# TencentYoutuResearch/ImageMatching-OETR

Hardware: AMD Instinct MI355X
Metric: image-pairs/sec @640x640 (OETR hot path: feature correlation + overlap regression, features resident in HBM) (higher is better)
Workload: dtype f32 (3xf16-split operands, fp32 accumulate); 1 GPU; BASELINE configs[1]: batch=8 pairs/GPU, 640x640 -> 20x20 tokens/image, C=256, 8 enc + 2 dec layers, f32_split_f16; pairs_per_gpu=8, global_pairs=8, streams=3, world_size=1, gpu_max_hw_queues=4, encoder_tile_rows=64, tail_mode=direct form (throughput setting for overlapped streams), parallelism=pairs sharded over 1 rank(s); all-gather of boxes only

## Files before the change

imagematching_oetr_amd/csrc/api.hip:

```cpp
#include <math.h>
#include <stdlib.h>
#include <string.h>

#include <string>
#include <vector>

#include "../../include/oetr_hip.h"
#include "common.h"

using namespace oetr;

constexpr int OETR_PREREDUCE_MIN_TOKENS = 768;
constexpr int OETR_DIRECT_TAIL_MIN_ROWS = 16000;

namespace {

thread_local std::string g_err;

oetr_status fail(oetr_status st, const std::string& msg) {
  g_err = msg;
  return st;
}
oetr_status hip_fail(hipError_t e, const char* what) {
  return fail(OETR_ERR_HIP, std::string(what) + ": " + hipGetErrorString(e));
// ... 97 lines not shown
    "k_decoder", "k_heat_conv", "k_heat_final", "k_size_reg", "k_boxes", "k_decoder_convp",
    "k_heat_combine", "k_neck_proj", "k_neck_conv", "k_neck_out", "k_kv_reduce"};

struct oetr_trace {
  std::vector<hipEvent_t> ev;
  std::vector<int> kid;
  int used = 0;
  int dropped = 0;
};

struct oetr_ctx {
  oetr_trace* trace = nullptr;
  int device = 0;
  int mode = GM_SPLIT;
  int kv_prereduce = -1;
  mutable int dec_fault = 0;
  int dec_split = 0;
  int tail_mode = 0;
  int policy = 0;
  int enc_tile = 0;
  int attn_full = 0;
  int num_cus = 256;
  float* dev = nullptr;
  size_t dev_floats = 0;
  EncLayerDev enc[OETR_N_ENC];
  DecKVDev dkv;
  DecLayerDev dec[OETR_N_DEC];
  const float* qe[2];
  const float *dec_tgt1, *dec_q0, *dec_qkv1;
  HeadsDev heads;
// ... 194 lines not shown

oetr_status run_correlation(oetr_ctx* h, const Geom& g, const Workspace& w, const float* feat1,
                            const float* feat2, const float* pos1, const float* pos2,
                            int enc_layers, hipStream_t s, bool with_decoder = true,
                            bool resident = false, const float* mask1 = nullptr,
                            const float* mask2 = nullptr) {
  EncLaunch p;
  memset(&p, 0, sizeof(p));
  if (!resident) {
    p.feat_nchw[0] = feat1; p.feat_nchw[1] = feat2;
    p.pos_nchw[0] = pos1; p.pos_nchw[1] = pos2;
    p.pos_out = w.pos;
  }
  p.tile_rows = encoder_tile_rows(h, g);
  p.g = encoder_geom(g, p.tile_rows);
#ifdef OETR_ABLATE
  { const char* e = getenv("OETR_ABLATE"); p.dbg = e ? atoi(e) : 0; }
#endif
#ifdef OETR_PHASE_TIMING
  {
    static long long* tb = nullptr;
    if (!tb) (void)hipMalloc(&tb, sizeof(long long) * 16 * 65536);
    p.tbuf = tb;
    g_tbuf = tb;
  }
#endif
  p.x = w.x; p.qp = w.qp; p.pos = w.pos;
  p.mask[0] = mask1; p.mask[1] = mask2;
  p.flags = w.flags;
  p.attn_full = h->attn_full;
  p.policy = h->policy;
  for (int i = 0; i < 2; ++i) p.lpad[i] = g.nt[i] * TM;
  p.vt_off[0] = 0; p.vt_off[1] = (size_t)g.N * C * p.lpad[0];
  p.kbuf_out = w.kbuf[0]; p.vt_out = w.vt[0];
  p.a = h->enc[0];
  p.kv_out = w.kvp[0]; p.ks_out = w.ksp[0];
  int prereduce = h->attn_full ? 0 : h->kv_prereduce;
  if (prereduce < 0) prereduce = (g.L[0] >= OETR_PREREDUCE_MIN_TOKENS || g.L[1] >= OETR_PREREDUCE_MIN_TOKENS) ? 1 : 0;
  TRACED(h, s, K_ENC_A, launch_encoder(p, false, 0, h->mode, s));
  p.feat_nchw[0] = p.feat_nchw[1] = p.pos_nchw[0] = p.pos_nchw[1] = nullptr;
  for (int l = 0; l < enc_layers; ++l) {
    p.b = h->enc[l];
    p.b_cross = l & 1;
    p.kv_in = w.kvp[l & 1]; p.ks_in = w.ksp[l & 1];
    p.kv_reduced = 0;
// ... 992 lines not shown
  (void)hipGetDevice(&prev);
  hipError_t e = hipSetDevice(device);
  if (e == hipSuccess) e = measure_mfma_rate(prop.multiProcessorCount, seconds, tflops, static_cast<hipStream_t>(stream));
  (void)hipSetDevice(prev);
  if (e != hipSuccess) return hip_fail(e, "oetr_debug_mfma_rate");
  return OETR_OK;
}

oetr_status oetr_set_state_prereduce(oetr_handle h, int on) {
  if (!h) return fail(OETR_ERR_BAD_ARG, "oetr_set_state_prereduce: NULL handle");
  if (on < -1 || on > 1) return fail(OETR_ERR_BAD_ARG, "oetr_set_state_prereduce: -1 (auto), 0 (off) or 1 (a reduction launch between the encoder launches)");
  h->kv_prereduce = on;
  return OETR_OK;
}

oetr_status oetr_set_attention(oetr_handle h, oetr_attention mode) {
  if (!h) return fail(OETR_ERR_BAD_ARG, "oetr_set_attention: NULL handle");
  if (mode != OETR_ATTENTION_LINEAR && mode != OETR_ATTENTION_FULL)
    return fail(OETR_ERR_BAD_ARG, "oetr_set_attention: unknown mode");
  if (mode == OETR_ATTENTION_FULL && h->policy != 0)
    return fail(OETR_ERR_UNSUPPORTED, "attention 'full' is not built for OETR_DTYPE_F32_SPLIT_QK16");
  if (mode == OETR_ATTENTION_FULL && !gm_f16_range(h->mode) && h->mode != GM_F32)
    return fail(OETR_ERR_UNSUPPORTED, "attention 'full' is built for OETR_DTYPE_F32_SPLIT_F16, OETR_DTYPE_F16 and OETR_DTYPE_F32");
  h->attn_full = mode == OETR_ATTENTION_FULL;
  return OETR_OK;
}

oetr_status oetr_set_trace(oetr_handle h, oetr_trace_handle t) {
  if (!h) return fail(OETR_ERR_BAD_ARG, "oetr_set_trace: NULL handle");
  h->trace = t;
// ... 39 lines not shown
```

imagematching_oetr_amd/csrc/common.h:

```cpp
#pragma once
#include <hip/hip_runtime.h>
#include <stdint.h>

#include <string>
#include <type_traits>

#include "../../include/oetr_hip.h"

namespace oetr {

constexpr int C = 256;
constexpr int NH = 8;
constexpr int HD = 32;
constexpr int FF = 512;
constexpr int TM = 32;
constexpr int LDA = C + 4;
constexpr int LDH = FF + 4;
constexpr int NTHREADS = 256;
constexpr int KV_FLOATS = NH * HD * HD;
constexpr float LN_EPS = 1e-5f;
constexpr float ATTN_EPS = 1e-6f;
constexpr int MAX_TOKENS = 10000;


// ... 818 lines not shown
  float* z0_out;
  float* dkv1_out;
  float* dks1_out;
  const float* dec_q0;
  EncLayerDev b;
  EncLayerDev a;
  DecKVDev d;
  int attn_full;
  const float* kbuf_in;
  const float* vt_in;
  float* kbuf_out;
  float* vt_out;
  int lpad[2];
  size_t vt_off[2];
  int tile_rows;
  int b_cross;
  int kv_reduced;
  int policy;
  int dbg;
  long long* tbuf;
  uint32_t* flags;
  const float* feat_nchw[2];
  const float* pos_nchw[2];
  float* pos_out;
  const float* mask[2];
};

hipError_t launch_encoder(const EncLaunch& p, bool has_b, int tail, int mode, hipStream_t s);
hipError_t launch_kv_reduce(const Geom& g, const float* kvp, const float* ksp, float* kvr, float* ksr,
                            hipStream_t s);

struct MhaDev {
  const float *wq_t, *wk_t, *wv_t, *wm_t;
  const float *bq, *bk, *bv;
};
struct DecLayerDev {
  MhaDev self_attn, cross;
  const float *w1_t, *w2_t;
  const float *n1w, *n1b, *n2w, *n2b, *n3w, *n3b;
};
struct DecLaunch {
  Geom g;
  DecLayerDev layer[2];
// ... 124 lines not shown
```

imagematching_oetr_amd/csrc/encoder.hip:

```cpp
#include <type_traits>

#include "common.h"


#ifndef OETR_SOAK_AMP
#define OETR_SOAK_AMP 0
#endif
#ifndef OETR_SPLIT_STATE
#define OETR_SPLIT_STATE 1
#endif

namespace oetr {

constexpr int S0_OFF = 0;
constexpr int S1_OFF = S0_OFF + TM * LDA;
constexpr int H_OFF = S1_OFF + TILE_FLOATS;
constexpr int KSUM_OFF = H_OFF + HID_FLOATS;
constexpr int Z_OFF = KSUM_OFF + C;
constexpr int LNP_OFF = Z_OFF + TM * NH;
constexpr int SMEM_FLOATS = LNP_OFF + 6 * C;

template <int NW>
struct EncCfg {
  static constexpr int NT = 8 / NW;
// ... 58 lines not shown
}

template <int THREADS>
__device__ __forceinline__ void load_tile(float* S, const float* __restrict__ src, int nvalid,
                                          int tid) {
#pragma unroll
  for (int i = 0; i < (TM * C / 4) / THREADS; ++i) {
    const int idx = tid + THREADS * i;
    const int r = idx >> 6, c4 = idx & 63;
    *reinterpret_cast<f32x4*>(S + r * LDA + 4 * c4) =
        reinterpret_cast<const f32x4*>(src + (size_t)min(r, nvalid - 1) * C)[c4];
  }
}

template <int THREADS, int ROWS>
__device__ __forceinline__ void load_tile_nchw(float* S, const float* __restrict__ src, int L,
                                               int nvalid, int tid) {
  constexpr int CG = THREADS / ROWS;
  const int r = tid % ROWS, cg = tid / ROWS;
  const float* s = src + min(r, nvalid - 1);
#pragma unroll
  for (int i = 0; i < C / CG; ++i) {
    const int c = cg + CG * i;
    S[r * LDA + c] = s[(size_t)c * L];
  }
}
template <int THREADS, int ROWS>
__device__ __forceinline__ void store_tile_tokens(float* __restrict__ dst, const float* S, int nvalid,
                                                  int tid) {
#pragma unroll
  for (int i = 0; i < (ROWS * C / 4) / THREADS; ++i) {
    const int idx = tid + THREADS * i;
    const int r = idx >> 6, c4 = idx & 63;
    if (r < nvalid)
      reinterpret_cast<f32x4*>(dst + (size_t)r * C)[c4] = *reinterpret_cast<const f32x4*>(S + r * LDA + 4 * c4);
  }
}

template <int MODE>
__device__ __forceinline__ void full_attention_tile(const EncLaunch& p, int n, int ss, size_t row_base,
// ... 594 lines not shown
    dec_layer(std::integral_constant<int, 1>{});
  }
  range_report<MODE>(rg, p.flags);
}

constexpr int LNX_LD = 36;
template <int RTW>
struct E2 {
  static constexpr int RFL = (2 * RTW * LDAH * 2 + 3) / 4;
  static_assert(RFL >= RTW * LDA, "region holds the f32 tile too");
  static constexpr int R1 = 0, R2 = RFL, KSUM = 2 * RFL, LNP = KSUM + C;
  static constexpr int LNX = LNP + 6 * C;
  static constexpr int SMEM = LNX + RTW * LNX_LD;
};

template <int MODE, int NMT = 2, bool MASKED = false>
__device__ __forceinline__ void kv_state_64(const f32x16 (&accK)[NMT], const f32x16 (&accV)[NMT],
                                            int S_len, int nvalid, int half, bool two, f32x16& kv,
                                            float& ksum, Range& rg, const float* msk_s = nullptr) {
  const float inv_len = 1.0f / (float)S_len;
  kv = f32x16{0};
  ksum = 0.f;
  int nv2 = nvalid - 4 * half;
  asm volatile("" : "+v"(nv2));
  if constexpr (MODE == GM_SPLIT && OETR_SPLIT_STATE) {
    f32x16 c1 = {0};
#if OETR_SOAK_AMP & 2
    __builtin_amdgcn_s_setprio(3);
#endif
    auto row_tile = [&](auto MT_) {
      constexpr int mt = decltype(MT_)::value;
#pragma unroll
      for (int st = 0; st < 2; ++st) {
        f32x4 k0, k1, v0, v1;
#pragma unroll
        for (int i = 0; i < 8; ++i) {
          const int r = 8 * st + i;
          float m;
          if constexpr (MASKED) m = msk_s[32 * mt + crow(r, half)];
          else m = 32 * mt + crow(r, 0) < nv2 ? 1.0f : 0.0f;
          const float kk = elu1(accK[mt][r]) * m;
          const float vv = accV[mt][r] * (inv_len * m);
          ksum += kk;
          if (i < 4) { k0[i] = kk; v0[i] = vv; } else { k1[i - 4] = kk; v1[i - 4] = vv; }
        }
        f32x4 ah, al, bh, bl;
        split8(k0, k1, ah, al, rg);
        split8(v0, v1, bh, bl, rg);
        mma16_split3(ah, al, bh, bl, kv, c1);
        __builtin_amdgcn_sched_barrier(0);
      }
    };
    row_tile(std::integral_constant<int, 0>{});
    if constexpr (NMT == 2) {
      if (two) row_tile(std::integral_constant<int, 1>{});
    }
#if OETR_SOAK_AMP & 2
    __builtin_amdgcn_s_setprio(0);
#endif
#pragma unroll
    for (int r = 0; r < 16; ++r) kv[r] = fmaf(c1[r], SPLIT_INV, kv[r]);
  } else {
    auto row_tile = [&](auto MT_) {
      constexpr int mt = decltype(MT_)::value;
      auto operands = [&](int r, float& k, float& v) {
        float m;
        if constexpr (MASKED) m = msk_s[32 * mt + crow(r, half)];
        else m = 32 * mt + crow(r, 0) < nv2 ? 1.0f : 0.0f;
        const float x = accK[mt][r];
        k = (elu1(x)) * m;
        ksum += k;
        v = accV[mt][r] * (inv_len * m);
      };
      float kc, vc;
      operands(0, kc, vc);
#pragma unroll
      for (int r = 0; r < 16; ++r) {
        float kn = 0.f, vn = 0.f;
        if (r + 1 < 16) operands(r + 1, kn, vn);
        kv = __builtin_amdgcn_mfma_f32_32x32x2f32(kc, vc, kv, 0, 0, 0);
        __builtin_amdgcn_sched_barrier(0);
        kc = kn; vc = vn;
// ... 4 lines not shown
      if (two) row_tile(std::integral_constant<int, 1>{});
    }
  }
  ksum += __shfl_xor(ksum, 32, 64);
}
__device__ __forceinline__ void kv_state_write(const f32x16& kv, float ksum, int lane, int wave,
                                               float* __restrict__ kv_out,
                                               float* __restrict__ ks_out, int slot) {
  f32x4* dst = reinterpret_cast<f32x4*>(kv_out) + ((size_t)slot * NH + wave) * 4 * 64;
#pragma unroll
  for (int q = 0; q < 4; ++q) {
    f32x4 o = {kv[4 * q], kv[4 * q + 1], kv[4 * q + 2], kv[4 * q + 3]};
    store16(reinterpret_cast<float*>(dst), (q * 64 + (unsigned)lane) * 16u, o);
  }
  if (lane < 32) (ks_out + (size_t)slot * C + wave * HD)[(unsigned)lane] = ksum;
}

template <bool HAS_B, int TAIL, int MODE, int POL, int ROWS, int RTW = RT, bool MASKED = false>
__device__ __forceinline__ void encoder64_body(const EncLaunch& p, float* smem) {
  constexpr int NMT = RTW / 32, THREADS = 512, TPR = THREADS / RTW, F4 = 64 / TPR;
  using L2 = E2<RTW>;
  using SP = SitePolicy<POL>;
  float* R1f = smem + L2::R1;
  float* R2f = smem + L2::R2;
  Range rg;
  const PlanesT<MODE, RTW> P1(R1f, &rg), P2(R2f, &rg);
  float* Xf = HAS_B ? R2f : R1f;
  float* ksum_s = smem + L2::KSUM;
  float* lnp_s = smem + L2::LNP;
  float* lnx_s = smem + L2::LNX;
  using WS = WStream2T<MODE, ROWS, NMT>;
  WS ws;
  constexpr int P_MERGE = 0;
  constexpr int P_1A = WS::adv(P_MERGE), P_1B = WS::adv(P_1A), P_2A = WS::adv(P_1B), P_2B = WS::adv(P_2A);
  constexpr int P_T0 = HAS_B ? WS::adv(P_2B) : 0;
  constexpr int P_T1 = WS::adv(P_T0), P_T2 = WS::adv(P_T1), P_T3 = WS::adv(P_T2);

  const Geom& g = p.g;
  const int tid = threadIdx.x, lane = tid & 63, wave = __builtin_amdgcn_readfirstlane(tid >> 6);
  const int half = lane >> 5, col = lane & 31;
  const int wcol = 32 * wave;
  const int lrow = tid / TPR, lpart = tid % TPR;

  const int logical = xcd_remap(blockIdx.x, g.ntiles);
  const int per = g.nt[0] + g.nt[1];
  const int n = logical / per;
  const int rem = logical - n * per;
  const int side = rem >= g.nt[0];
  const int t_idx = side ? rem - g.nt[0] : rem;
  const int L = g.L[side];
  const int l0 = t_idx * RTW;
  const int nvalid = min(RTW, L - l0);
  const size_t row_base = (size_t)g.row0[side] + (size_t)n * L + l0;
  const int slot = g.tile0[side] + n * g.nt[side] + t_idx;
  const size_t qrow_base = (size_t)slot * RTW;
  const bool nchw = !HAS_B && p.feat_nchw[0] != nullptr;
  ws.set_rows(nvalid);
  ws.set_lane(lane);

  stage_ln_params<THREADS, HAS_B, TAIL>(lnp_s, p, tid);
  const f32x4* pos = reinterpret_cast<const f32x4*>(
                         p.pos + (size_t)(g.prow0[side] + l0 + min(lrow, nvalid - 1)) * C) + lpart;

  f32x16 xacc[NMT];
  PHASE_STAMP(p, 0);
  if (!HAS_B) PHASE_STAMP(p, 13);

  if (HAS_B) {
    const int ss = p.b_cross ? 1 - side : side;
    const int S_len = g.L[ss];
    const int nts = p.kv_reduced ? 1 : g.nt[ss];
    const int src_slot0 = p.kv_reduced ? ss * g.N + n : g.tile0[ss] + n * g.nt[ss];

    f32x4 kvB[4];
#pragma unroll
    for (int q = 0; q < 4; ++q) kvB[q] = f32x4{0.f, 0.f, 0.f, 0.f};
    {
      constexpr int KVR = 7;
      const unsigned ln = lane, kl = tid & (C - 1);
      const f32x4* kvp = reinterpret_cast<const f32x4*>(p.kv_in) + ((size_t)src_slot0 * NH + wave) * 256;
      const float* ksp = p.ks_in + (size_t)src_slot0 * C;
      float ks = 0.f;
      if (nts == 1) {
#pragma unroll
        for (int e = 0; e < 4; ++e) kvB[e] = kvp[e * 64 + ln];
        ks = ksp[kl];
      } else
      for (int ti0 = 0; ti0 < nts; ti0 += KVR) {
        f32x4 tmp[KVR][4];
// ... 3 lines not shown
          const int ti = min(ti0 + u, nts - 1);
#pragma unroll
          for (int e = 0; e < 4; ++e) tmp[u][e] = kvp[(size_t)ti * (NH * 256) + e * 64 + ln];
          kt[u] = ksp[(size_t)ti * C + kl];
        }
#pragma unroll
        for (int u = 0; u < KVR; ++u)
          if (ti0 + u < nts) {
#pragma unroll
            for (int e = 0; e < 4; ++e) kvB[e] += tmp[u][e];
            ks += kt[u];
          }
      }
      if (tid < C) ksum_s[tid] = ks;
    }
    ws.template prime<C, P_MERGE, SP::MERGE>(p.b.wmerge, p.b.wmerge_l, wave, 0, lane);
    f32x4 qfrag[NMT][4];
    {
      const f32x4* qf = reinterpret_cast<const f32x4*>(p.qp + qrow_base * C) + (size_t)wave * NMT * 4 * 64;
#pragma unroll
      for (int mt = 0; mt < NMT; ++mt)
#pragma unroll
        for (int u = 0; u < 4; ++u) qfrag[mt][u] = qf[(mt * 4 + u) * 64 + (unsigned)lane];
    }
#pragma unroll
    for (int mt = 0; mt < NMT; ++mt) {
      const float* xr = p.x + (row_base + min(32 * mt + col, nvalid - 1)) * C + wcol + 4 * half;
#pragma unroll
      for (int g4 = 0; g4 < 4; ++g4) {
        const f32x4 v = *reinterpret_cast<const f32x4*>(xr + 8 * g4);
#pragma unroll
        for (int i = 0; i < 4; ++i) xacc[mt][4 * g4 + i] = v[i];
      }
    }
    __syncthreads();
    PHASE_STAMP(p, 1);

    {
      f32x4 kvh[2], kvl[2], ksh[2], ksl[2];
      const float inv_S = 1.0f / (float)S_len;
      (void)inv_S;
      if constexpr (gm_f16_range(MODE)) {
#pragma unroll
        for (int s2 = 0; s2 < 2; ++s2) {
          split8(kvB[2 * s2], kvB[2 * s2 + 1], kvh[s2], kvl[s2], rg);
          const float* kr = ksum_s + wave * HD + 4 * half + 16 * s2;
          split8(*reinterpret_cast<const f32x4*>(kr) * inv_S, *reinterpret_cast<const f32x4*>(kr + 8) * inv_S,
                 ksh[s2], ksl[s2], rg);
        }
      }
#pragma unroll
      for (int mt = 0; mt < NMT; ++mt) {
        if (mt == 1 && !ws.two()) break;
        f32x16 macc = {0}, zacc = {0};
        if constexpr (gm_f16_range(MODE)) {
          f32x16 c1 = {0}, cz = {0};
#pragma unroll
          for (int s2 = 0; s2 < 2; ++s2) {
            const f32x4 qh = qfrag[mt][2 * s2], ql = qfrag[mt][2 * s2 + 1];
            mma16_split3(kvh[s2], kvl[s2], qh, ql, macc, c1);
            mma16_split3(ksh[s2], ksl[s2], qh, ql, zacc, cz);
          }
#pragma unroll
          for (int r = 0; r < 16; ++r) macc[r] = fmaf(c1[r], SPLIT_INV, macc[r]);
          zacc[0] = fmaf(cz[0], SPLIT_INV, zacc[0]);
        } else {
#pragma unroll
          for (int ks4 = 0; ks4 < 4; ++ks4) {
            const f32x4 q = qfrag[mt][ks4];
            const f32x4 kk = *reinterpret_cast<const f32x4*>(ksum_s + wave * HD + 4 * half + ks4 * 8);
#pragma unroll
            for (int j = 0; j < 4; ++j) {
              macc = __builtin_amdgcn_mfma_f32_32x32x2f32(kvB[ks4][j], q[j], macc, 0, 0, 0);
              zacc = __builtin_amdgcn_mfma_f32_32x32x2f32(kk[j], q[j], zacc, 0, 0, 0);
            }
          }
        }
        const float zdot = gm_f16_range(MODE) ? zacc[0] * (float)S_len : zacc[0];
        const float zs = (float)S_len / (zdot + ATTN_EPS);
#pragma unroll
        for (int g4 = 0; g4 < 4; ++g4)
          P1.put4(32 * mt + col, wcol + 8 * g4 + 4 * half,
                  f32x4{macc[4 * g4] * zs, macc[4 * g4 + 1] * zs, macc[4 * g4 + 2] * zs, macc[4 * g4 + 3] * zs});
      }
    }
    __syncthreads();
    PHASE_STAMP(p, 2);

    ws.template gemm<C, P_MERGE, true, C, SP::MERGE, SP::MLP1, true>(P1, p.b.wmerge, p.b.wmerge_l, wave, 0, lane,
                                                                     xacc, p.b.w1, p.b.w1_l, wave, 0);
    PHASE_STAMP(p, 3);
    {
      float pm[NMT], pq[NMT];
#pragma unroll
// ... 72 lines not shown
      PHASE_STAMP(p, 7);
      ws.template gemm<FF, P_2B, (TAIL != 2), C, SP::MLP2, SNEXT, XTR>(P1, p.b.w2, p.b.w2_l, wave, 16, lane, xacc,
                                                                       TAIL == 0 ? p.a.wq : p.d.wk[0],
                                                                       TAIL == 0 ? p.a.wq_l : p.d.wk_l[0], wave, 0);
    }
#pragma unroll
    for (int mt = 0; mt < NMT; ++mt)
#pragma unroll
      for (int g4 = 0; g4 < 4; ++g4)
        *reinterpret_cast<f32x4*>(Xf + (32 * mt + col) * LDA + wcol + 8 * g4 + 4 * half) =
            f32x4{xacc[mt][4 * g4], xacc[mt][4 * g4 + 1], xacc[mt][4 * g4 + 2], xacc[mt][4 * g4 + 3]};
    __syncthreads();
#pragma unroll
    for (int i = 0; i < RTW / 8; ++i) {
      const int r = wave + 8 * i;
      if (r < nvalid)
        store16(p.x + (row_base + r) * C, 16u * (unsigned)lane,
                                    *reinterpret_cast<const f32x4*>(Xf + r * LDA + 4 * lane));
    }
    PHASE_STAMP(p, 8);
    if (TAIL == 2) { range_report<MODE>(rg, p.flags); return; }
  } else {
    if (nchw) {
      load_tile_nchw<THREADS, RTW>(R1f, p.feat_nchw[side] + (size_t)n * C * L + l0, L, nvalid, tid);
      load_tile_nchw<THREADS, RTW>(R2f, p.pos_nchw[side] + l0, L, nvalid, tid);
    } else {
#pragma unroll
      for (int i = 0; i < (RTW * C / 4) / THREADS; ++i) {
        const int idx = tid + THREADS * i;
        const int r = idx >> 6, c4 = idx & 63;
        *reinterpret_cast<f32x4*>(R1f + r * LDA + 4 * c4) =
            reinterpret_cast<const f32x4*>(p.x + (row_base + min(r, nvalid - 1)) * C)[c4];
      }
    }
    if (TAIL == 0) ws.template prime<C, P_T0, SP::Q>(p.a.wq, p.a.wq_l, wave, 0, lane);
    if (TAIL == 1) ws.template prime<C, P_T0, SP::DEC_K>(p.d.wk[0], p.d.wk_l[0], wave, 0, lane);
    __syncthreads();
    if (nchw) {
      store_tile_tokens<THREADS, RTW>(p.x + row_base * C, R1f, nvalid, tid);
      if (n == 0) store_tile_tokens<THREADS, RTW>(p.pos_out + (size_t)(g.prow0[side] + l0) * C, R2f, nvalid, tid);
    }
    PHASE_STAMP(p, 14);
  }

  if constexpr (MASKED && TAIL != 2) {
    if (tid < RTW) lnx_s[tid] = tid < nvalid ? p.mask[side][(size_t)n * L + l0 + tid] : 0.f;
  }
  if (TAIL == 0) {
    {
      f32x4 xn[F4], ps[F4];
      if (!HAS_B && nchw) {
        const f32x4* pl = reinterpret_cast<const f32x4*>(R2f + lrow * LDA) + lpart;
#pragma unroll
        for (int i = 0; i < F4; ++i) ps[i] = pl[i * TPR];
      } else {
#pragma unroll
        for (int i = 0; i < F4; ++i) ps[i] = pos[i * TPR];
      }
      ln_rows<TPR, F4>(Xf, tid, xn, 0);
      __syncthreads();
// ... 12 lines not shown
    PHASE_STAMP(p, 9);
    f32x16 accQ[NMT] = {};
    ws.template gemm<C, P_T0, true, C, SP::Q, SP::K, true>(P1, p.a.wq, p.a.wq_l, wave, 0, lane, accQ, p.a.wk,
                                                           p.a.wk_l, wave, 0);
    PHASE_STAMP(p, 10);
    f32x16 accK[NMT] = {}, accV[NMT] = {};
    {
      f32x4* qf = reinterpret_cast<f32x4*>(p.qp + qrow_base * C) + (size_t)wave * NMT * 4 * 64;
      const bool two = ws.two();
      u32x4 qhi = {0, 0, 0, 0}, qlo = {0, 0, 0, 0};
      auto qepi = [&](auto CI_) {
        constexpr int CI = decltype(CI_)::value, mt = NMT == 2 ? CI / 8 : 0, pr = NMT == 2 ? CI % 8 : CI / 2;
        constexpr int s2 = pr / 4, j = pr % 4;
        if constexpr (NMT == 1 && CI % 2 == 1) return;
        if (mt == 1 && !two) return;
        const float qmask = MASKED ? lnx_s[32 * mt + col] : 1.0f;
        const float a = MASKED ? elu1(accQ[mt][2 * pr]) * qmask : elu1(accQ[mt][2 * pr]);
        const float b = MASKED ? elu1(accQ[mt][2 * pr + 1]) * qmask : elu1(accQ[mt][2 * pr + 1]);
        if constexpr (MODE == GM_BF16) {
          if constexpr (pr % 2 == 0) { qhi[0] = __builtin_bit_cast(uint32_t, a); qhi[1] = __builtin_bit_cast(uint32_t, b); }
          else {
            qhi[2] = __builtin_bit_cast(uint32_t, a); qhi[3] = __builtin_bit_cast(uint32_t, b);
            store16(reinterpret_cast<float*>(qf), ((mt * 4 + pr / 2) * 64 + (unsigned)lane) * 16u,
                                        __builtin_bit_cast(f32x4, qhi));
          }
        } else {
          uint32_t h, l;
          cvt_planes2<GM_SPLIT>(a, b, h, l, rg);
          qhi[j] = h; qlo[j] = l;
          if constexpr (j == 3) {
            store16(reinterpret_cast<float*>(qf), ((mt * 4 + 2 * s2) * 64 + (unsigned)lane) * 16u,
// ... 1 lines not shown
            store16(reinterpret_cast<float*>(qf), ((mt * 4 + 2 * s2 + 1) * 64 + (unsigned)lane) * 16u,
                                        __builtin_bit_cast(f32x4, qlo));
          }
        }
      };
      ws.template gemm_epi<C, P_T1, true, C, SP::K, SP::V>(P2, p.a.wk, p.a.wk_l, wave, 0, lane, accK, p.a.wv,
                                                           p.a.wv_l, wave, 0, qepi);
    }
    ws.template gemm<C, P_T2, false, C, SP::V>(P2, p.a.wv, p.a.wv_l, wave, 0, lane, accV, nullptr, nullptr,
                                               0, 0);
    PHASE_STAMP(p, 11);
    f32x16 kv;
    float ksum;
    kv_state_64<MODE, NMT, MASKED>(accK, accV, L, nvalid, half, ws.two(), kv, ksum, rg, lnx_s);
    kv_state_write(kv, ksum, lane, wave, p.kv_out, p.ks_out, slot);
    PHASE_STAMP(p, 12);
  } else if (TAIL == 1) {
    float bias_k[2], bias_v[2];
#pragma unroll
    for (int dl = 0; dl < 2; ++dl) {
      bias_k[dl] = p.d.bk[dl][wcol + col];
      bias_v[dl] = p.d.bv[dl][wcol + col];
    }
    {
      f32x4 xv[F4], ps[F4];
      const f32x4* src = reinterpret_cast<const f32x4*>(Xf + lrow * LDA) + lpart;
#pragma unroll
      for (int i = 0; i < F4; ++i) { xv[i] = src[i * TPR]; ps[i] = pos[i * TPR]; }
      __syncthreads();
#pragma unroll
// ... 5 lines not shown
    __syncthreads();
    auto dec_layer = [&](auto DL) {
      constexpr int dl = decltype(DL)::value;
      constexpr int PK = dl == 0 ? P_T0 : P_T2, PV = dl == 0 ? P_T1 : P_T3;
      f32x16 accK[NMT], accV[NMT];
#pragma unroll
      for (int mt = 0; mt < NMT; ++mt)
#pragma unroll
        for (int r = 0; r < 16; ++r) { accK[mt][r] = bias_k[dl]; accV[mt][r] = bias_v[dl]; }
      ws.template gemm<C, PK, true, C, SP::DEC_K, SP::DEC_V>(P1, p.d.wk[dl], p.d.wk_l[dl], wave, 0, lane, accK,
                                                             p.d.wv[dl], p.d.wv_l[dl], wave, 0);
      ws.template gemm<C, PV, false, C, SP::DEC_V>(P2, p.d.wv[dl], p.d.wv_l[dl], wave, 0, lane, accV, nullptr,
                                                   nullptr, 0, 0);
      f32x16 kv;
      float ksum;
      kv_state_64<MODE, NMT, MASKED>(accK, accV, L, nvalid, half, ws.two(), kv, ksum, rg, lnx_s);
      if constexpr (dl == 1) {
        kv_state_write(kv, ksum, lane, wave, p.dkv1_out, p.dks1_out, slot);
      } else {
        const float* q0 = p.dec_q0 + side * C + wave * HD;
        float a = 0.f;
#pragma unroll
        for (int r = 0; r < 16; ++r) a += q0[crow(r, half)] * kv[r];
        a += __shfl_xor(a, 32, 64);
        float z = q0[col] * ksum;
        z += __shfl_xor(z, 1, 64);
        z += __shfl_xor(z, 2, 64);
        z += __shfl_xor(z, 4, 64);
        z += __shfl_xor(z, 8, 64);
        z += __shfl_xor(z, 16, 64);
        if (half == 0) p.att0_out[(size_t)slot * C + wave * HD + col] = a;
        if (lane == 0) p.z0_out[(size_t)slot * NH + wave] = z;
        ws.template prime<C, P_T2, SP::DEC_K>(p.d.wk[1], p.d.wk_l[1], wave, 0, lane);
      }
    };
    dec_layer(std::integral_constant<int, 0>{});
    dec_layer(std::integral_constant<int, 1>{});
  }
  range_report<MODE>(rg, p.flags);
}

template <bool HAS_B, int TAIL, int MODE, int POL = 0, bool MASKED = false>
__global__ __launch_bounds__(512) void k_encoder64(EncLaunch p) {
  __shared__ __attribute__((aligned(16))) float smem[E2<RT>::SMEM];
  if constexpr (gm_planes(MODE) == 2) {
    const Geom& g = p.g;
    const int logical = xcd_remap(blockIdx.x, g.ntiles);
    const int per = g.nt[0] + g.nt[1];
    const int rem = logical - (logical / per) * per;
    const int side = rem >= g.nt[0];
    const int t_idx = side ? rem - g.nt[0] : rem;
    const int nvalid = min(RT, g.L[side] - t_idx * RT);
    if (__builtin_amdgcn_readfirstlane(nvalid > 32 ? 1 : 0)) encoder64_body<HAS_B, TAIL, MODE, POL, 2, RT, MASKED>(p, smem);
    else encoder64_body<HAS_B, TAIL, MODE, POL, 1, RT, MASKED>(p, smem);
  } else {
    encoder64_body<HAS_B, TAIL, MODE, POL, 0, RT, MASKED>(p, smem);
  }
}

template <bool HAS_B, int TAIL, int MODE, int POL = 0, bool MASKED = false>
__global__ __launch_bounds__(512) void k_encoder32m(EncLaunch p) {
  __shared__ __attribute__((aligned(16))) float smem[E2<TM>::SMEM];
  encoder64_body<HAS_B, TAIL, MODE, POL, 2, TM, MASKED>(p, smem);
}

template <int NOB_TAIL_MAX, class F>
static hipError_t launch_b_tail(bool has_b, int tail, F launch) {
// ... 2 lines not shown
  constexpr std::integral_constant<int, 2> t2{};
  if (has_b) {
    if (tail == 0) launch(std::true_type{}, t0);
    else if (tail == 1) launch(std::true_type{}, t1);
    else launch(std::true_type{}, t2);
  } else {
    if (tail == 0) launch(std::false_type{}, t0);
    else if constexpr (NOB_TAIL_MAX == 0) return hipErrorInvalidValue;
    else if (tail == 1) launch(std::false_type{}, t1);
    else if constexpr (NOB_TAIL_MAX == 1) return hipErrorInvalidValue;
    else launch(std::false_type{}, t2);
  }
  return hipGetLastError();
}

template <int MODE>
static hipError_t launch_encoder_mode(const EncLaunch& p, bool has_b, int tail, hipStream_t s) {
  const dim3 grid(p.g.ntiles);
  if (p.mask[0] || p.mask[1]) {
    if constexpr (MODE == GM_SPLIT) {
      if (!p.mask[0] || !p.mask[1] || (p.policy != 0 && p.policy != 1) || p.attn_full) return hipErrorInvalidValue;
      return launch_b_tail<0>(has_b, tail, [&](auto b, auto t) {
        if (p.policy == 1) {
          if (p.tile_rows == RT) hipLaunchKernelGGL((k_encoder64<b(), t(), MODE, 1, true>), grid, dim3(512), 0, s, p);
          else hipLaunchKernelGGL((k_encoder32m<b(), t(), MODE, 1, true>), grid, dim3(512), 0, s, p);
        } else {
          if (p.tile_rows == RT) hipLaunchKernelGGL((k_encoder64<b(), t(), MODE, 0, true>), grid, dim3(512), 0, s, p);
          else hipLaunchKernelGGL((k_encoder32m<b(), t(), MODE, 0, true>), grid, dim3(512), 0, s, p);
        }
      });
    } else if constexpr (MODE == GM_F32) {
      if (!p.mask[0] || !p.mask[1] || p.policy != 0 || p.attn_full) return hipErrorInvalidValue;
      return launch_b_tail<0>(has_b, tail, [&](auto b, auto t) {
// ... 99 lines not shown
```

imagematching_oetr_amd/hip_engine.py:

```python
import ctypes as C
import os
import time
from pathlib import Path

import torch

_PKG_DIR = Path(__file__).resolve().parent
LIB_PATH = _PKG_DIR / 'csrc' / 'liboetr_hip.so'

N_ENC, N_DEC, D_MODEL, N_HEAD = 8, 2, 256, 8
_f32p = C.POINTER(C.c_float)


class _EncW(C.Structure):
    _fields_ = [(n, _f32p) for n in (
        'q_proj', 'k_proj', 'v_proj', 'merge', 'mlp0', 'mlp2',
        'pre_norm_q_w', 'pre_norm_q_b', 'pre_norm_kv_w', 'pre_norm_kv_b',
        'norm2_w', 'norm2_b')]


class _MhaW(C.Structure):
    _fields_ = [(n, _f32p) for n in (
        'q_proj_w', 'q_proj_b', 'k_proj_w', 'k_proj_b', 'v_proj_w',
        'v_proj_b', 'merge')]
# ... 54 lines not shown
    'oetr_size_regression', 'oetr_box_tlbr_to_xyxy', 'oetr_linear_attention',
    'oetr_full_attention', 'oetr_trace_create', 'oetr_trace_destroy',
    'oetr_set_trace', 'oetr_trace_summary', 'oetr_neck_create',
    'oetr_neck_destroy', 'oetr_neck_workspace_bytes', 'oetr_neck_forward',
    'oetr_neck_set_trace', 'oetr_set_encoder_tile', 'oetr_query_flags',
    'oetr_neck_query_flags', 'oetr_overlap_crop', 'oetr_overlap_crop_capacity',
    'oetr_full_attention_split', 'oetr_set_attention', 'oetr_neck_set_conv_rows',
    'oetr_linear_attention_workspace_bytes', 'oetr_neck_set_conv_kernel',
    'oetr_token_buffers', 'oetr_forward_tokens', 'oetr_neck_forward_tokens',
    'oetr_workspace_init', 'oetr_read_flags_async', 'oetr_neck_read_flags_async',
    'oetr_set_state_prereduce', 'oetr_set_tail_mode', 'oetr_set_decoder_split', 'oetr_overlap_frame', 'oetr_read_overlap_image',
    'oetr_forward_masked', 'oetr_feature_correlation_masked', 'oetr_center_estimation_masked',
    'oetr_linear_attention_masked', 'oetr_debug_decoder_fault',
    'oetr_flagslot_device_pointer', 'oetr_forward_flagslot', 'oetr_forward_tokens_flagslot',
    'oetr_neck_forward_tokens_status', 'oetr_debug_mfma_rate')

FLAG_F16_RANGE = 1
FLAG_EXCHANGE = 2
FLAG_INVALID = FLAG_F16_RANGE | FLAG_EXCHANGE
FLAG_PUBLISHED = 0x80000000

BANK_ABI_VERSION = 1
BANK_EXPORTS = ('oetr_bank_abi_version', 'oetr_bank_gather', 'oetr_forward_bank')
FLAG_INDEX = 4

COVIS_ABI_VERSION = 1
COVIS_EXPORTS = ('oetr_covis_abi_version', 'oetr_covis_workspace_bytes', 'oetr_covis_boxes')
COVIS_PARAM_DOUBLES = 40

COVIS_SET_ABI_VERSION = 1
# ... 116 lines not shown
    lib.oetr_trace_create.restype = i
    lib.oetr_trace_create.argtypes = [i, C.POINTER(vp)]
    lib.oetr_trace_destroy.restype = None
    lib.oetr_trace_destroy.argtypes = [vp]
    lib.oetr_set_trace.restype = i
    lib.oetr_set_trace.argtypes = [vp, vp]
    lib.oetr_trace_summary.restype = i
    lib.oetr_trace_summary.argtypes = [vp, C.POINTER(i), C.POINTER(C.c_char_p),
                                       C.POINTER(i), C.POINTER(C.c_float)]
    lib.oetr_set_encoder_tile.restype = i
    lib.oetr_set_encoder_tile.argtypes = [vp, i]
    lib.oetr_set_attention.restype = i
    lib.oetr_set_attention.argtypes = [vp, i]
    lib.oetr_set_state_prereduce.restype = i
    lib.oetr_set_state_prereduce.argtypes = [vp, i]
    lib.oetr_set_tail_mode.restype = i
    lib.oetr_set_tail_mode.argtypes = [vp, i]
    lib.oetr_set_decoder_split.restype = i
    lib.oetr_set_decoder_split.argtypes = [vp, i]
    lib.oetr_debug_decoder_fault.restype = i
    lib.oetr_debug_decoder_fault.argtypes = [vp, i]
    lib.oetr_neck_create.restype = i
    lib.oetr_neck_create.argtypes = [C.POINTER(_NeckWeights), i, C.POINTER(vp)]
    lib.oetr_neck_destroy.restype = None
    lib.oetr_neck_destroy.argtypes = [vp]
    lib.oetr_neck_workspace_bytes.restype = sz
    lib.oetr_neck_workspace_bytes.argtypes = [vp, i, i, i]
    lib.oetr_neck_forward.restype = i
    lib.oetr_neck_forward.argtypes = [vp, vp, i, i, i, vp, sz, vp, vp]
    lib.oetr_neck_forward_tokens.restype = i
# ... 355 lines not shown
            self.set_state_prereduce(int(os.environ['OETR_STATE_PREREDUCE']))

    __del__ = _destructor('oetr_destroy')

    def set_encoder_tile(self, rows):
        _check(self.lib, self.lib.oetr_set_encoder_tile(self._h, int(rows or 0)),
               'oetr_set_encoder_tile')
        self._enc_tile_set = int(rows or 0)

    def _current_ws(self):
        return self._ws.get(torch.cuda.current_stream(self.device).cuda_stream)

    def set_state_prereduce(self, mode):
        _check(self.lib, self.lib.oetr_set_state_prereduce(self._h, int(mode)), 'oetr_set_state_prereduce')

    def set_tail_mode(self, mode):
        _check(self.lib, self.lib.oetr_set_tail_mode(self._h, int(mode)), 'oetr_set_tail_mode')
        self._tail_mode_set = int(mode)

    def set_decoder_split(self, k):
        _check(self.lib, self.lib.oetr_set_decoder_split(self._h, int(k)), 'oetr_set_decoder_split')
        self._dec_split_set = int(k)

    def debug_decoder_fault(self, on=True):
        _check(self.lib, self.lib.oetr_debug_decoder_fault(self._h, int(bool(on))), 'oetr_debug_decoder_fault')

    def settle_exchange(self):
        ws = self._current_ws()
        if ws is not None:
            with torch.cuda.device(self.device):
# ... 593 lines not shown
```

Measured before the change: 33780 image-pairs/s.

## Pack both images' partial tail tiles into one shared encoder workgroup

When both images' token counts leave a remainder of at most 16 rows in the last 64-row tile, the two partial tail tiles of a pair are merged into a single workgroup. Each half of the 32-row tile belongs to a different image and uses its own attention state, KV/ksum reduction and output slot. This removes one mostly-empty workgroup per pair, freeing CU slots for the overlapped streams. The cost is extra MMA and state-reduction work, plus more complex indexing, in every one-row-tile body, and the merged workgroup takes longer to finish.

```diff
diff --git a/imagematching_oetr_amd/csrc/api.hip b/imagematching_oetr_amd/csrc/api.hip
--- a/imagematching_oetr_amd/csrc/api.hip
+++ b/imagematching_oetr_amd/csrc/api.hip
@@ -2,10 +2,12 @@
 #include <stdlib.h>
 #include <string.h>
 
+#include <atomic>
 #include <string>
 #include <vector>
 
 #include "../../include/oetr_hip.h"
+#include "../../include/oetr_tail_share.h"
 #include "common.h"
 
 using namespace oetr;
@@ -135,6 +137,8 @@
   int device = 0;
   int mode = GM_SPLIT;
   int kv_prereduce = -1;
+  int tail_share = -1;
+  mutable std::atomic<int> enc_grid{0};
   mutable int dec_fault = 0;
   int dec_split = 0;
   int tail_mode = 0;
@@ -359,6 +363,9 @@
   }
   p.tile_rows = encoder_tile_rows(h, g);
   p.g = encoder_geom(g, p.tile_rows);
+  p.tail_share = h->tail_share != 0;
+  p.attn_full = h->attn_full;
+  h->enc_grid.store(encoder_workgroups(p, h->mode), std::memory_order_relaxed);
 #ifdef OETR_ABLATE
   { const char* e = getenv("OETR_ABLATE"); p.dbg = e ? atoi(e) : 0; }
 #endif
@@ -373,7 +380,6 @@
   p.x = w.x; p.qp = w.qp; p.pos = w.pos;
   p.mask[0] = mask1; p.mask[1] = mask2;
   p.flags = w.flags;
-  p.attn_full = h->attn_full;
   p.policy = h->policy;
   for (int i = 0; i < 2; ++i) p.lpad[i] = g.nt[i] * TM;
   p.vt_off[0] = 0; p.vt_off[1] = (size_t)g.N * C * p.lpad[0];
@@ -1396,6 +1402,15 @@
   return OETR_OK;
 }
 
+oetr_status oetr_set_tail_share(oetr_handle h, int mode) {
+  if (!h) return fail(OETR_ERR_BAD_ARG, "oetr_set_tail_share: NULL handle");
+  if (mode != -1 && mode != 0) return fail(OETR_ERR_BAD_ARG, "oetr_set_tail_share: -1 (auto) or 0 (off)");
+  h->tail_share = mode;
+  return OETR_OK;
+}
+
+int oetr_debug_encoder_grid(oetr_handle h) { return h ? h->enc_grid.load(std::memory_order_relaxed) : -1; }
+
 oetr_status oetr_set_attention(oetr_handle h, oetr_attention mode) {
   if (!h) return fail(OETR_ERR_BAD_ARG, "oetr_set_attention: NULL handle");
   if (mode != OETR_ATTENTION_LINEAR && mode != OETR_ATTENTION_FULL)
diff --git a/imagematching_oetr_amd/csrc/common.h b/imagematching_oetr_amd/csrc/common.h
--- a/imagematching_oetr_amd/csrc/common.h
+++ b/imagematching_oetr_amd/csrc/common.h
@@ -856,6 +856,8 @@
   int lpad[2];
   size_t vt_off[2];
   int tile_rows;
+  int nwg;
+  int tail_share;
   int b_cross;
   int kv_reduced;
   int policy;
@@ -869,6 +871,7 @@
 };
 
 hipError_t launch_encoder(const EncLaunch& p, bool has_b, int tail, int mode, hipStream_t s);
+int encoder_workgroups(const EncLaunch& p, int mode);
 hipError_t launch_kv_reduce(const Geom& g, const float* kvp, const float* ksp, float* kvr, float* ksr,
                             hipStream_t s);
 
diff --git a/imagematching_oetr_amd/csrc/encoder.hip b/imagematching_oetr_amd/csrc/encoder.hip
--- a/imagematching_oetr_amd/csrc/encoder.hip
+++ b/imagematching_oetr_amd/csrc/encoder.hip
@@ -96,16 +96,19 @@
 }
 
 template <int THREADS, int ROWS>
-__device__ __forceinline__ void load_tile_nchw(float* S, const float* __restrict__ src, int L,
-                                               int nvalid, int tid) {
+__device__ __forceinline__ void load_rows_nchw(float* S, const float* __restrict__ s, int L, int tid) {
   constexpr int CG = THREADS / ROWS;
   const int r = tid % ROWS, cg = tid / ROWS;
-  const float* s = src + min(r, nvalid - 1);
 #pragma unroll
   for (int i = 0; i < C / CG; ++i) {
     const int c = cg + CG * i;
     S[r * LDA + c] = s[(size_t)c * L];
   }
+}
+template <int THREADS, int ROWS>
+__device__ __forceinline__ void load_tile_nchw(float* S, const float* __restrict__ src, int L,
+                                               int nvalid, int tid) {
+  load_rows_nchw<THREADS, ROWS>(S, src + min(tid % ROWS, nvalid - 1), L, tid);
 }
 template <int THREADS, int ROWS>
 __device__ __forceinline__ void store_tile_tokens(float* __restrict__ dst, const float* S, int nvalid,
@@ -730,7 +733,7 @@
   static constexpr int SMEM = LNX + RTW * LNX_LD;
 };
 
-template <int MODE, int NMT = 2, bool MASKED = false>
+template <int MODE, int NMT = 2, bool MASKED = false, bool LO16 = false>
 __device__ __forceinline__ void kv_state_64(const f32x16 (&accK)[NMT], const f32x16 (&accV)[NMT],
                                             int S_len, int nvalid, int half, bool two, f32x16& kv,
                                             float& ksum, Range& rg, const float* msk_s = nullptr) {
@@ -754,6 +757,7 @@
           const int r = 8 * st + i;
           float m;
           if constexpr (MASKED) m = msk_s[32 * mt + crow(r, half)];
+          else if constexpr (LO16) m = (r >= 8 && 32 * mt + crow(r, 0) < nv2) ? 1.0f : 0.0f;
           else m = 32 * mt + crow(r, 0) < nv2 ? 1.0f : 0.0f;
           const float kk = elu1(accK[mt][r]) * m;
           const float vv = accV[mt][r] * (inv_len * m);
@@ -782,6 +786,7 @@
       auto operands = [&](int r, float& k, float& v) {
         float m;
         if constexpr (MASKED) m = msk_s[32 * mt + crow(r, half)];
+        else if constexpr (LO16) m = (r >= 8 && 32 * mt + crow(r, 0) < nv2) ? 1.0f : 0.0f;
         else m = 32 * mt + crow(r, 0) < nv2 ? 1.0f : 0.0f;
         const float x = accK[mt][r];
         k = (elu1(x)) * m;
@@ -816,6 +821,21 @@
     store16(reinterpret_cast<float*>(dst), (q * 64 + (unsigned)lane) * 16u, o);
   }
   if (lane < 32) (ks_out + (size_t)slot * C + wave * HD)[(unsigned)lane] = ksum;
+}
+
+struct EncWg { int n, side, t_idx; bool shared; };
+__device__ __forceinline__ EncWg enc_wg(const EncLaunch& p) {
+  const Geom& g = p.g;
+  const int logical = xcd_remap(blockIdx.x, p.nwg);
+  const int f0 = g.nt[0] - p.tail_share;
+  const int per = f0 + g.nt[1];
+  EncWg w;
+  w.n = logical / per;
+  const int rem = logical - w.n * per;
+  w.shared = p.tail_share != 0 && rem == per - 1;
+  w.side = !w.shared && rem >= f0;
+  w.t_idx = w.shared ? f0 : w.side ? rem - f0 : rem;
+  return w;
 }
 
 template <bool HAS_B, int TAIL, int MODE, int POL, int ROWS, int RTW = RT, bool MASKED = false>
@@ -831,6 +851,7 @@
   float* ksum_s = smem + L2::KSUM;
   float* lnp_s = smem + L2::LNP;
   float* lnx_s = smem + L2::LNX;
+  float* ksum2_s = lnx_s + 32 * LNX_LD;
   using WS = WStream2T<MODE, ROWS, NMT>;
   WS ws;
   constexpr int P_MERGE = 0;
@@ -844,12 +865,8 @@
   const int wcol = 32 * wave;
   const int lrow = tid / TPR, lpart = tid % TPR;
 
-  const int logical = xcd_remap(blockIdx.x, g.ntiles);
-  const int per = g.nt[0] + g.nt[1];
-  const int n = logical / per;
-  const int rem = logical - n * per;
-  const int side = rem >= g.nt[0];
-  const int t_idx = side ? rem - g.nt[0] : rem;
+  const EncWg wg = enc_wg(p);
+  const int n = wg.n, side = wg.side, t_idx = wg.t_idx;
   const int L = g.L[side];
   const int l0 = t_idx * RTW;
   const int nvalid = min(RTW, L - l0);
@@ -860,9 +877,21 @@
   ws.set_rows(nvalid);
   ws.set_lane(lane);
 
+  constexpr bool Seg2 = ROWS == 1 && RTW == RT;
+  static_assert(!Seg2 || gm_f16_range(MODE), "one-row-tile body: two-plane modes");
+  const int r2 = Seg2 && wg.shared ? g.L[1] - (g.nt[1] - 1) * RTW : 0;
+  const bool sh = r2 != 0;
+  const int side2 = sh ? 1 : side, Lb = g.L[side2], l02 = sh ? (g.nt[1] - 1) * RTW : l0;
+  const size_t row_base2 = sh ? (size_t)g.row0[1] + (size_t)n * Lb + l02 : row_base;
+  const int slot2 = sh ? g.tile0[1] + n * g.nt[1] + g.nt[1] - 1 : slot;
+  auto seg_of = [&](int r) { return Seg2 && sh && r >= 16; };
+  auto seg_row = [&](int r) { return seg_of(r) ? min(r - 16, r2 - 1) : min(r, nvalid - 1); };
+  auto x_row = [&](int r) { return (seg_of(r) ? row_base2 : row_base) + seg_row(r); };
+  auto pos_row = [&](int r) { return (seg_of(r) ? g.prow0[1] + l02 : g.prow0[side] + l0) + seg_row(r); };
+  const bool lane_seg = seg_of(col);
+
   stage_ln_params<THREADS, HAS_B, TAIL>(lnp_s, p, tid);
-  const f32x4* pos = reinterpret_cast<const f32x4*>(
-                         p.pos + (size_t)(g.prow0[side] + l0 + min(lrow, nvalid - 1)) * C) + lpart;
+  const f32x4* pos = reinterpret_cast<const f32x4*>(p.pos + (size_t)pos_row(lrow) * C) + lpart;
 
   f32x16 xacc[NMT];
   PHASE_STAMP(p, 0);
@@ -875,6 +904,7 @@
     const int src_slot0 = p.kv_reduced ? ss * g.N + n : g.tile0[ss] + n * g.nt[ss];
 
     f32x4 kvB[4];
+    auto reduce_state = [&](f32x4 (&kvB)[4], float* ksum_s, int nts, int src_slot0) {
 #pragma unroll
     for (int q = 0; q < 4; ++q) kvB[q] = f32x4{0.f, 0.f, 0.f, 0.f};
     {
@@ -908,6 +938,20 @@
       }
       if (tid < C) ksum_s[tid] = ks;
     }
+    };
+    reduce_state(kvB, ksum_s, nts, src_slot0);
+    const int ss2 = p.b_cross ? 1 - side2 : side2;
+    const int S_len2 = g.L[ss2];
+    f32x4 kvB2[4];
+    if constexpr (Seg2) {
+      if (sh) {
+        reduce_state(kvB2, ksum2_s, p.kv_reduced ? 1 : g.nt[ss2], p.kv_reduced ? ss2 * g.N + n : g.tile0[ss2] + n * g.nt[ss2]);
+      } else {
+#pragma unroll
+        for (int q = 0; q < 4; ++q) kvB2[q] = f32x4{0.f, 0.f, 0.f, 0.f};
+        if (tid < C) ksum2_s[tid] = 0.f;
+      }
+    }
     ws.template prime<C, P_MERGE, SP::MERGE>(p.b.wmerge, p.b.wmerge_l, wave, 0, lane);
     f32x4 qfrag[NMT][4];
     {
@@ -919,7 +963,7 @@
     }
 #pragma unroll
     for (int mt = 0; mt < NMT; ++mt) {
-      const float* xr = p.x + (row_base + min(32 * mt + col, nvalid - 1)) * C + wcol + 4 * half;
+      const float* xr = p.x + x_row(32 * mt + col) * C + wcol + 4 * half;
 #pragma unroll
       for (int g4 = 0; g4 < 4; ++g4) {
         const f32x4 v = *reinterpret_cast<const f32x4*>(xr + 8 * g4);
@@ -932,6 +976,7 @@
 
     {
       f32x4 kvh[2], kvl[2], ksh[2], ksl[2];
+      f32x4 kvh2[2], kvl2[2], ksh2[2], ksl2[2];
       const float inv_S = 1.0f / (float)S_len;
       (void)inv_S;
       if constexpr (gm_f16_range(MODE)) {
@@ -941,6 +986,13 @@
           const float* kr = ksum_s + wave * HD + 4 * half + 16 * s2;
           split8(*reinterpret_cast<const f32x4*>(kr) * inv_S, *reinterpret_cast<const f32x4*>(kr + 8) * inv_S,
                  ksh[s2], ksl[s2], rg);
+          if constexpr (Seg2) {
+            const float inv_S2 = 1.0f / (float)S_len2;
+            split8(kvB2[2 * s2], kvB2[2 * s2 + 1], kvh2[s2], kvl2[s2], rg);
+            const float* kr2 = ksum2_s + wave * HD + 4 * half + 16 * s2;
+            split8(*reinterpret_cast<const f32x4*>(kr2) * inv_S2, *reinterpret_cast<const f32x4*>(kr2 + 8) * inv_S2,
+                   ksh2[s2], ksl2[s2], rg);
+          }
         }
       }
 #pragma unroll
@@ -958,6 +1010,18 @@
 #pragma unroll
           for (int r = 0; r < 16; ++r) macc[r] = fmaf(c1[r], SPLIT_INV, macc[r]);
           zacc[0] = fmaf(cz[0], SPLIT_INV, zacc[0]);
+          if constexpr (Seg2) {
+            f32x16 macc2 = {0}, zacc2 = {0}, c2 = {0}, cz2 = {0};
+#pragma unroll
+            for (int s2 = 0; s2 < 2; ++s2) {
+              const f32x4 qh = qfrag[mt][2 * s2], ql = qfrag[mt][2 * s2 + 1];
+              mma16_split3(kvh2[s2], kvl2[s2], qh, ql, macc2, c2);
+              mma16_split3(ksh2[s2], ksl2[s2], qh, ql, zacc2, cz2);
+            }
+#pragma unroll
+            for (int r = 0; r < 16; ++r) macc[r] = lane_seg ? fmaf(c2[r], SPLIT_INV, macc2[r]) : macc[r];
+            zacc[0] = lane_seg ? fmaf(cz2[0], SPLIT_INV, zacc2[0]) : zacc[0];
+          }
         } else {
 #pragma unroll
           for (int ks4 = 0; ks4 < 4; ++ks4) {
@@ -970,8 +1034,9 @@
             }
           }
         }
-        const float zdot = gm_f16_range(MODE) ? zacc[0] * (float)S_len : zacc[0];
-        const float zs = (float)S_len / (zdot + ATTN_EPS);
+        const float S_lane = lane_seg ? (float)S_len2 : (float)S_len;
+        const float zdot = gm_f16_range(MODE) ? zacc[0] * S_lane : zacc[0];
+        const float zs = S_lane / (zdot + ATTN_EPS);
 #pragma unroll
         for (int g4 = 0; g4 < 4; ++g4)
           P1.put4(32 * mt + col, wcol + 8 * g4 + 4 * half,
@@ -1074,36 +1139,64 @@
 #pragma unroll
     for (int i = 0; i < RTW / 8; ++i) {
       const int r = wave + 8 * i;
-      if (r < nvalid)
-        store16(p.x + (row_base + r) * C, 16u * (unsigned)lane,
+      if (seg_of(r) ? r - 16 < r2 : r < nvalid)
+        store16(p.x + x_row(r) * C, 16u * (unsigned)lane,
                                     *reinterpret_cast<const f32x4*>(Xf + r * LDA + 4 * lane));
     }
     PHASE_STAMP(p, 8);
     if (TAIL == 2) { range_report<MODE>(rg, p.flags); return; }
   } else {
     if (nchw) {
+      if constexpr (Seg2) {
+        const int r = tid % RTW;
+        const bool s2 = seg_of(r);
+        const int Ls = s2 ? Lb : L, tok = (s2 ? l02 : l0) + seg_row(r);
+        load_rows_nchw<THREADS, RTW>(R1f, p.feat_nchw[s2 ? 1 : side] + (size_t)n * C * Ls + tok, Ls, tid);
+        load_rows_nchw<THREADS, RTW>(R2f, p.pos_nchw[s2 ? 1 : side] + tok, Ls, tid);
+      } else {
       load_tile_nchw<THREADS, RTW>(R1f, p.feat_nchw[side] + (size_t)n * C * L + l0, L, nvalid, tid);
       load_tile_nchw<THREADS, RTW>(R2f, p.pos_nchw[side] + l0, L, nvalid, tid);
+      }
     } else {
 #pragma unroll
       for (int i = 0; i < (RTW * C / 4) / THREADS; ++i) {
         const int idx = tid + THREADS * i;
         const int r = idx >> 6, c4 = idx & 63;
         *reinterpret_cast<f32x4*>(R1f + r * LDA + 4 * c4) =
-            reinterpret_cast<const f32x4*>(p.x + (row_base + min(r, nvalid - 1)) * C)[c4];
+            reinterpret_cast<const f32x4*>(p.x + x_row(r) * C)[c4];
       }
     }
     if (TAIL == 0) ws.template prime<C, P_T0, SP::Q>(p.a.wq, p.a.wq_l, wave, 0, lane);
     if (TAIL == 1) ws.template prime<C, P_T0, SP::DEC_K>(p.d.wk[0], p.d.wk_l[0], wave, 0, lane);
     __syncthreads();
     if (nchw) {
+      if constexpr (Seg2) {
+#pragma unroll
+        for (int i = 0; i < 32 / 8; ++i) {
+          const int r = wave + 8 * i;
+          if (seg_of(r) ? r - 16 < r2 : r < nvalid) {
+            reinterpret_cast<f32x4*>(p.x + x_row(r) * C)[lane] = *reinterpret_cast<const f32x4*>(R1f + r * LDA + 4 * lane);
+            if (n == 0)
+              reinterpret_cast<f32x4*>(p.pos_out + (size_t)pos_row(r) * C)[lane] = *reinterpret_cast<const f32x4*>(R2f + r * LDA + 4 * lane);
+          }
+        }
+      } else {
       store_tile_tokens<THREADS, RTW>(p.x + row_base * C, R1f, nvalid, tid);
       if (n == 0) store_tile_tokens<THREADS, RTW>(p.pos_out + (size_t)(g.prow0[side] + l0) * C, R2f, nvalid, tid);
+      }
     }
     PHASE_STAMP(p, 14);
   }
 
-  if constexpr (MASKED && TAIL != 2) {
+  if constexpr (MASKED && TAIL != 2 && Seg2) {
+    if (tid < 32) {
+      const bool s2 = seg_of(tid);
+      const bool ok = s2 ? tid - 16 < r2 : tid < nvalid;
+      const float m = ok ? p.mask[s2 ? 1 : side][(size_t)n * (s2 ? Lb : L) + (s2 ? l02 : l0) + seg_row(tid)] : 0.f;
+      lnx_s[tid] = s2 ? 0.f : m;
+      lnx_s[32 + tid] = s2 ? m : 0.f;
+    }
+  } else if constexpr (MASKED && TAIL != 2) {
     if (tid < RTW) lnx_s[tid] = tid < nvalid ? p.mask[side][(size_t)n * L + l0 + tid] : 0.f;
   }
   if (TAIL == 0) {
@@ -1146,7 +1239,7 @@
         constexpr int s2 = pr / 4, j = pr % 4;
         if constexpr (NMT == 1 && CI % 2 == 1) return;
         if (mt == 1 && !two) return;
-        const float qmask = MASKED ? lnx_s[32 * mt + col] : 1.0f;
+        const float qmask = MASKED ? lnx_s[32 * (Seg2 ? (int)lane_seg : mt) + col] : 1.0f;
         const float a = MASKED ? elu1(accQ[mt][2 * pr]) * qmask : elu1(accQ[mt][2 * pr]);
         const float b = MASKED ? elu1(accQ[mt][2 * pr + 1]) * qmask : elu1(accQ[mt][2 * pr + 1]);
         if constexpr (MODE == GM_BF16) {
@@ -1178,6 +1271,10 @@
     float ksum;
     kv_state_64<MODE, NMT, MASKED>(accK, accV, L, nvalid, half, ws.two(), kv, ksum, rg, lnx_s);
     kv_state_write(kv, ksum, lane, wave, p.kv_out, p.ks_out, slot);
+    if constexpr (Seg2) {
+      kv_state_64<MODE, NMT, MASKED, true>(accK, accV, Lb, 16 + r2, half, false, kv, ksum, rg, lnx_s + 32);
+      if (sh) kv_state_write(kv, ksum, lane, wave, p.kv_out, p.ks_out, slot2);
+    }
     PHASE_STAMP(p, 12);
   } else if (TAIL == 1) {
     float bias_k[2], bias_v[2];
@@ -1213,11 +1310,11 @@
                                                    nullptr, 0, 0);
       f32x16 kv;
       float ksum;
-      kv_state_64<MODE, NMT, MASKED>(accK, accV, L, nvalid, half, ws.two(), kv, ksum, rg, lnx_s);
+      auto emit = [&](int side_, int slot_, bool on) {
       if constexpr (dl == 1) {
-        kv_state_write(kv, ksum, lane, wave, p.dkv1_out, p.dks1_out, slot);
+        if (on) kv_state_write(kv, ksum, lane, wave, p.dkv1_out, p.dks1_out, slot_);
       } else {
-        const float* q0 = p.dec_q0 + side * C + wave * HD;
+        const float* q0 = p.dec_q0 + side_ * C + wave * HD;
         float a = 0.f;
 #pragma unroll
         for (int r = 0; r < 16; ++r) a += q0[crow(r, half)] * kv[r];
@@ -1228,10 +1325,17 @@
         z += __shfl_xor(z, 4, 64);
         z += __shfl_xor(z, 8, 64);
         z += __shfl_xor(z, 16, 64);
-        if (half == 0) p.att0_out[(size_t)slot * C + wave * HD + col] = a;
-        if (lane == 0) p.z0_out[(size_t)slot * NH + wave] = z;
-        ws.template prime<C, P_T2, SP::DEC_K>(p.d.wk[1], p.d.wk_l[1], wave, 0, lane);
-      }
+        if (on && half == 0) p.att0_out[(size_t)slot_ * C + wave * HD + col] = a;
+        if (on && lane == 0) p.z0_out[(size_t)slot_ * NH + wave] = z;
+      }
+      };
+      kv_state_64<MODE, NMT, MASKED>(accK, accV, L, nvalid, half, ws.two(), kv, ksum, rg, lnx_s);
+      emit(side, slot, true);
+      if constexpr (Seg2) {
+        kv_state_64<MODE, NMT, MASKED, true>(accK, accV, Lb, 16 + r2, half, false, kv, ksum, rg, lnx_s + 32);
+        emit(side2, slot2, sh);
+      }
+      if constexpr (dl == 0) ws.template prime<C, P_T2, SP::DEC_K>(p.d.wk[1], p.d.wk_l[1], wave, 0, lane);
     };
     dec_layer(std::integral_constant<int, 0>{});
     dec_layer(std::integral_constant<int, 1>{});
@@ -1243,13 +1347,8 @@
 __global__ __launch_bounds__(512) void k_encoder64(EncLaunch p) {
   __shared__ __attribute__((aligned(16))) float smem[E2<RT>::SMEM];
   if constexpr (gm_planes(MODE) == 2) {
-    const Geom& g = p.g;
-    const int logical = xcd_remap(blockIdx.x, g.ntiles);
-    const int per = g.nt[0] + g.nt[1];
-    const int rem = logical - (logical / per) * per;
-    const int side = rem >= g.nt[0];
-    const int t_idx = side ? rem - g.nt[0] : rem;
-    const int nvalid = min(RT, g.L[side] - t_idx * RT);
+    const EncWg wg = enc_wg(p);
+    const int nvalid = min(RT, p.g.L[wg.side] - wg.t_idx * RT);
     if (__builtin_amdgcn_readfirstlane(nvalid > 32 ? 1 : 0)) encoder64_body<HAS_B, TAIL, MODE, POL, 2, RT, MASKED>(p, smem);
     else encoder64_body<HAS_B, TAIL, MODE, POL, 1, RT, MASKED>(p, smem);
   } else {
@@ -1282,9 +1381,21 @@
   return hipGetLastError();
 }
 
+static bool encoder_tail_share(const EncLaunch& p, int mode) {
+  if (!p.tail_share || mode != GM_SPLIT || p.tile_rows != RT || p.attn_full) return false;
+  const int r1 = p.g.L[0] % RT, r2 = p.g.L[1] % RT;
+  return r1 >= 1 && r1 <= 16 && r2 >= 1 && r2 <= 16;
+}
+int encoder_workgroups(const EncLaunch& p, int mode) {
+  return p.g.ntiles - (encoder_tail_share(p, mode) ? p.g.N : 0);
+}
+
 template <int MODE>
-static hipError_t launch_encoder_mode(const EncLaunch& p, bool has_b, int tail, hipStream_t s) {
-  const dim3 grid(p.g.ntiles);
+static hipError_t launch_encoder_mode(const EncLaunch& p_in, bool has_b, int tail, hipStream_t s) {
+  EncLaunch p = p_in;
+  p.tail_share = encoder_tail_share(p_in, MODE) ? 1 : 0;
+  p.nwg = encoder_workgroups(p_in, MODE);
+  const dim3 grid(p.nwg);
   if (p.mask[0] || p.mask[1]) {
     if constexpr (MODE == GM_SPLIT) {
       if (!p.mask[0] || !p.mask[1] || (p.policy != 0 && p.policy != 1) || p.attn_full) return hipErrorInvalidValue;
diff --git a/imagematching_oetr_amd/hip_engine.py b/imagematching_oetr_amd/hip_engine.py
--- a/imagematching_oetr_amd/hip_engine.py
+++ b/imagematching_oetr_amd/hip_engine.py
@@ -92,6 +92,7 @@
     'oetr_linear_attention_masked', 'oetr_debug_decoder_fault',
     'oetr_flagslot_device_pointer', 'oetr_forward_flagslot', 'oetr_forward_tokens_flagslot',
     'oetr_neck_forward_tokens_status', 'oetr_debug_mfma_rate')
+TAIL_SHARE_EXPORTS = ('oetr_set_tail_share', 'oetr_debug_encoder_grid')
 
 FLAG_F16_RANGE = 1
 FLAG_EXCHANGE = 2
@@ -238,6 +239,10 @@
     lib.oetr_set_attention.argtypes = [vp, i]
     lib.oetr_set_state_prereduce.restype = i
     lib.oetr_set_state_prereduce.argtypes = [vp, i]
+    lib.oetr_set_tail_share.restype = i
+    lib.oetr_set_tail_share.argtypes = [vp, i]
+    lib.oetr_debug_encoder_grid.restype = i
+    lib.oetr_debug_encoder_grid.argtypes = [vp]
     lib.oetr_set_tail_mode.restype = i
     lib.oetr_set_tail_mode.argtypes = [vp, i]
     lib.oetr_set_decoder_split.restype = i
@@ -623,6 +628,12 @@
     def set_state_prereduce(self, mode):
         _check(self.lib, self.lib.oetr_set_state_prereduce(self._h, int(mode)), 'oetr_set_state_prereduce')
 
+    def set_tail_share(self, mode):
+        _check(self.lib, self.lib.oetr_set_tail_share(self._h, int(mode)), 'oetr_set_tail_share')
+
+    def debug_encoder_grid(self):
+        return int(self.lib.oetr_debug_encoder_grid(self._h))
+
     def set_tail_mode(self, mode):
         _check(self.lib, self.lib.oetr_set_tail_mode(self._h, int(mode)), 'oetr_set_tail_mode')
         self._tail_mode_set = int(mode)
diff --git a/include/oetr_tail_share.h b/include/oetr_tail_share.h
--- /dev/null
+++ b/include/oetr_tail_share.h
@@ -0,0 +1,18 @@
+#ifndef OETR_TAIL_SHARE_H_
+#define OETR_TAIL_SHARE_H_
+
+#include "oetr_hip.h"
+
+#ifdef __cplusplus
+extern "C" {
+#endif
+
+oetr_status oetr_set_tail_share(oetr_handle h, int mode);
+
+int oetr_debug_encoder_grid(oetr_handle h);
+
+#ifdef __cplusplus
+}
+#endif
+
+#endif
```

Result: faster. 34800 image-pairs/s, median of 6 (+3.0%).
